# sholtodouglas/RoboticsPlayroomPybullet

Hardware: AMD Instinct MI355X
Metric: env-steps/sec at N=4096 parallel UR5PlayAbsRPY1Obj-v0 envs per MI355X (higher is better)
Workload: dtype f32

## Files before the change

### roboticsplayroompybullet_amd/csrc/rp_kernels.cuh

```cuda
#pragma once
#include <hip/hip_runtime.h>
#include <stdint.h>

#include "rp_device_model.h"
#include "rp_math.cuh"

#define NB_MAX (1 + RP_MAX_ARM + RP_MAX_FREE + RP_MAX_J1)
#define NVP 28
#define MAXC 21
#define MAXACT 64
#define MAXT 4
#define MAXROWC (3 * MAXC + MAXT)
static_assert(MAXACT <= 64 && NB_MAX <= 32, "a candidate record packs its pair index in 6 bits and its bodies in 5 bits each");
#define PM_MAX 11
#define PMC_HDR 4
#define PMC_PT 11
#define PMC_MAN (8 + 4 * PMC_PT)
#define PMC_MANIFOLDS (PMC_HDR + PM_MAX * PMC_MAN)
#define PMC_AX PMC_MANIFOLDS
#define PMC_AXN 16
#define PMC_FLOATS (PMC_MANIFOLDS + 8 * PMC_AXN)
#define RP_MAX_GROUPS 16
#define SORT_KEYS 64
#define SORT_REPS 8
// ... 103 lines not shown
  int act[MAXACT], candn[MAXACT], key[MAXACT];
  float pmu[MAXACT];
  alignas(16) float cand[CANDMAX * 8];
  alignas(16) float Minv[144];
  float tau[RP_MAX_ARM];
  float finv[RP_MAX_FREE * 9];
  float dmu[RP_MAX_OBJ], dmass[RP_MAX_FREE + 1];
  float vstar[32];
  union alignas(16) {
    struct {
      float inert[RP_MAX_ARM * 10], compI[RP_MAX_ARM * 10];
      float vsp[RP_MAX_ARM * 6], csp[RP_MAX_ARM * 6], fsp[RP_MAX_ARM * 6], Fv[RP_MAX_ARM * 6];
      double Md[144];
    };
    struct {
      float srow[MAXSMALL * 8];
      float rowS[3 * PREP_CH * 4], rowT[3 * PREP_CH * 4];
      union {
        struct { float J[3 * PREP_CH * ROWW], B[3 * PREP_CH * ROWW]; };
        float aout[192];
      };
    };
  };
  HULL_POOL_FIELDS
#ifdef RP_LDS_PAD
  float pad[RP_LDS_PAD];
#endif
};
static_assert(offsetof(EnvLds, aabb) % 16 == 0 && offsetof(PrepLds, aabb) % 16 == 0 && offsetof(EnvLds, cand) % 16 == 0 && offsetof(EnvLds, man) % 16 == 0 && offsetof(EnvLds, srow) % 16 == 0 && offsetof(EnvLds, rowS) % 16 == 0 &&
              offsetof(EnvLds, rowT) % 16 == 0 && offsetof(EnvLds, J) % 16 == 0 && offsetof(EnvLds, B) % 16 == 0, "16-byte LDS accesses");
static_assert(sizeof(PrepLds) <= 20480 - 512, "k_prep2: eight blocks (sixteen waves: what its 128 VGPRs allow) per CU");
static_assert(offsetof(PrepLds, roff) % 16 == 0 && offsetof(PrepLds, slot) % 16 == 0 && offsetof(PrepLds, Minv) % 16 == 0 && offsetof(PrepLds, aout) % 16 == 0 &&
              offsetof(PrepLds, Md) % 8 == 0 && offsetof(PrepLds, cand) % 16 == 0 && offsetof(PrepLds, man) % 16 == 0, "16-byte copies out of LDS");

struct __align__(16) ObsLds {
  float st[RP_REC_FLOATS];
  float xR[NB_MAX * 9], xp[NB_MAX * 3];
  float O[4];
  float S[RP_MAX_ARM * 6];
  alignas(16) float cand[2 * 12 * RP_MAX_ARM + 2 * RP_MAX_ARM + 4];
  alignas(16) float out[O_FLOATS];
};
#ifdef RP_CLOCKS
__device__ unsigned long long g_clk[32 * 4096];
#define CLK_MARK(i) if (lane == 0) { g_clk[8 * wb + (i)] = __builtin_readcyclecounter(); }
#if RP_CLOCKS == 2
#define PCLK(i) if (lane == 0) { g_clk[32 * (blockIdx.x & 4095) + (i)] = (i) >= 6 && (i) < 8 ? wall_clock64() : __builtin_readcyclecounter(); }
#define PCLK_ZERO(i) if (lane == 0) { g_clk[32 * (blockIdx.x & 4095) + (i)] = 0ull; }
#define PCLK_ADD(i, v) if (lane == 0) { g_clk[32 * (blockIdx.x & 4095) + (i)] += (unsigned long long)(v); }
#define HCLK_ADD(i, v) if (l16 == 0) { atomicAdd(&g_clk[32 * (blockIdx.x & 4095) + (i)], (unsigned long long)(v)); }
#ifdef RP_HPROF
#define PCLK_G(i, v)
#define PCLK_H(i, v) PCLK_ADD(i, v)
#else
#define PCLK_G(i, v) PCLK_ADD(i, v)
#define PCLK_H(i, v)
#endif
#define CLK_MARK2(i)
#else
#define PCLK(i)
#define PCLK_ZERO(i)
#define PCLK_ADD(i, v)
#define HCLK_ADD(i, v)
#define PCLK_G(i, v)
#define PCLK_H(i, v)
#define CLK_MARK2(i) CLK_MARK(i)
// ... 108 lines not shown

__device__ __forceinline__ Xf joint_compose(const DevModel* m, const Xf& P, int j, float q) {
  Xf r;
  M3 Rj = mul(P.R, ldm3(m->arm_jrot[j]));
  r.p = P.p + mulv(P.R, ld3(m->arm_jpos[j]));
  V3 ax = ld3(m->arm_axis[j]);
  if (m->arm_jtype[j] == 0) {
    r.R = mul(Rj, axis_angle(ax, q));
  } else {
    r.R = Rj;
    r.p = r.p + mulv(Rj, ax) * q;
  }
  return r;
}

template <class LDS>
__device__ __forceinline__ void fk_bodies(const DevModel* m, LDS& L, int lane) {
  float* T = L.cand;
  static_assert(2 * 12 * RP_MAX_ARM + 2 * RP_MAX_ARM <= CANDMAX * 8 && 2 * 12 * RP_MAX_ARM + 2 * RP_MAX_ARM <= (int)(sizeof(L.cand) / sizeof(float)), "fk scratch fits the candidate list");
  int* P = (int*)(T + 2 * 12 * RP_MAX_ARM);
  const int n = m->n_arm;
  Xf x; x.R = ident3(); x.p = mk3(0, 0, 0);
  int par = -1;
  if (lane < n) {
    M3 R0 = ldm3(m->arm_jrot[lane]);
    V3 p0 = ld3(m->arm_jpos[lane]), ax = ld3(m->arm_axis[lane]);
    float q = L.st[ST_Q + lane];
    x.R = R0; x.p = p0;
    if (m->arm_jtype[lane] == 0) x.R = mul(R0, axis_angle(ax, q));
    else x.p = p0 + mulv(R0, ax) * q;
    par = m->arm_parent[lane];
    if (par < 0) { M3 Rb = ldm3(m->base_rot); V3 pb = ld3(m->base_pos); x.p = pb + mulv(Rb, x.p); x.R = mul(Rb, x.R); }
  }
  for (int it = 0; __ballot(par >= 0) != 0ull; it++) {
    float* Tb = T + (it & 1) * 12 * RP_MAX_ARM;
    int* Pb = P + (it & 1) * RP_MAX_ARM;
    if (lane < n) { stm3(&Tb[12 * lane], x.R); st3(&Tb[12 * lane + 9], x.p); Pb[lane] = par; }
    WSYNC();
    if (par >= 0) {
      M3 Ra = ldm3(&Tb[12 * par]); V3 pa = ld3(&Tb[12 * par + 9]);
      x.p = pa + mulv(Ra, x.p); x.R = mul(Ra, x.R);
      par = Pb[par];
    }
  }
  if (lane < n) { stm3(&L.xR[9 * (lane + 1)], x.R); st3(&L.xp[3 * (lane + 1)], x.p); }
  if (lane < m->nbody && !(lane >= 1 && lane <= n)) {
    int b = lane;
    Xf y; y.R = ident3(); y.p = mk3(0, 0, 0);
    if (b > n && b <= n + m->n_free) {
      int k = b - 1 - n;
      const float* f = &L.st[ST_FREE + 13 * k];
      Q4 q = {f[3], f[4], f[5], f[6]};
      y.R = quat_to_m3(q); y.p = ld3(f);
    } else if (b > n + m->n_free) {
      int k = b - 1 - n - m->n_free;
      M3 R0 = ldm3(m->j1_rot[k]);
      V3 ax = ld3(m->j1_axis[k]);
      y.p = ld3(m->j1_pos[k]);
      float q = L.st[ST_JQ + k];
      if (m->j1_type[k] == 0) y.R = mul(R0, axis_angle(ax, q));
      else { y.R = R0; y.p = y.p + mulv(R0, ax) * q; }
    }
    stm3(&L.xR[9 * b], y.R); st3(&L.xp[3 * b], y.p);
  }
}

template <class LDS>
__device__ __forceinline__ void joint_subspaces(const DevModel* m, LDS& L, int lane) {
  if (lane == 0) st3(L.O, ld3(&L.xp[3 * m->site_body[RP_SITE_EE]]));
  WSYNC();
  if (lane < m->n_arm) {
    V3 O = ld3(L.O);
    M3 R = ldm3(&L.xR[9 * (1 + lane)]);
    V3 a = mulv(R, ld3(m->arm_axis[lane]));
    V6 S;
    if (m->arm_jtype[lane] == 0) { S.a = a; S.l = cross(ld3(&L.xp[3 * (1 + lane)]) - O, a); }
    else { S.a = mk3(0, 0, 0); S.l = a; }
    st6(&L.S[6 * lane], S);
  }
}

template <class LDS>
__device__ __forceinline__ void stage_dynamics(const DevModel* m, LDS& L, int t, int env) {
  const int no = m->n_obj, nd = no + m->n_free;
  if (t < nd) {
    const float v = m->dyn[(size_t)env * nd + t];
    if (t < no) L.dmu[t] = v; else L.dmass[t - no] = v;
  }
}
template <class LDS>
__device__ __forceinline__ float pair_friction(const DevModel* m, const LDS& L, int a, int b) {
  return fminf(L.dmu[m->col_obj[a]] * L.dmu[m->col_obj[b]], 10.f);
}
__device__ __forceinline__ V3 ld_wrench(const DevModel* m, int env, int body, int half) {
  return ld3(m->wrench + ((size_t)env * (m->nbody - 1) + body) * 6 + 3 * half);
}
__device__ __forceinline__ bool wrench_on(V3 w) { return w.x != 0.f || w.y != 0.f || w.z != 0.f; }
// ... 965 lines not shown
#pragma unroll
    for (int bit = 0; bit < 3; bit++) {
      const unsigned long long mb = __ballot((npl >> bit) & 1);
      off += __popcll(mb & lower_groups) << bit; tot += __popcll(mb) << bit;
    }
    cbase += tot;
    const int npg = __shfl(np, lane & ~7);
    const int nst = min(npg, max(0, CANDMAX - off));
    if (act && s < nst) {
      float* c = &L.cand[(off + s) * 8];
      *(float4*)c = make_float4(mine.p.x, mine.p.y, mine.p.z, mine.n.x);
      *(float4*)(c + 4) = make_float4(mine.n.y, mine.n.z, mine.dist, __int_as_float(a | (b << 8) | (ai << 16) | (body_a << 22) | (body_b << 27)));
    }
    if (act && s == 0) L.candn[ai] = nst | (min(off, CANDMAX) << 8);
    WSYNC();
  }
  return min(cbase, CANDMAX);
}

__device__ __forceinline__ int manifold_replace_index(const float* c4, const float* pt) {
  int deepest = -1; float maxpen = pt[6];
  for (int i = 0; i < 4; i++) if (c4[8 * i + 6] < maxpen - K_TIE_EPS) { deepest = i; maxpen = c4[8 * i + 6]; }
  float res[4] = {0, 0, 0, 0};
  V3 P = ld3(pt), p0 = ld3(c4), p1 = ld3(c4 + 8), p2 = ld3(c4 + 16), p3 = ld3(c4 + 24), cr;
  if (deepest != 0) { cr = cross(P - p1, p3 - p2); res[0] = dot(cr, cr); }
  if (deepest != 1) { cr = cross(P - p0, p3 - p2); res[1] = dot(cr, cr); }
  if (deepest != 2) { cr = cross(P - p0, p3 - p1); res[2] = dot(cr, cr); }
  if (deepest != 3) { cr = cross(P - p0, p2 - p1); res[3] = dot(cr, cr); }
  int best = 0;
  for (int i = 1; i < 4; i++) if (res[i] > res[best] * (1.f + 1e-4f)) best = i;
  return best;
}

template <class LDS>
__device__ __forceinline__ int collide(const DevModel* m, LDS& L, int lane, int env, const int* npm_early = nullptr) {
  int nact = 0;
  const int npair = m->n_pair;
  const unsigned short* pp = (const unsigned short*)m->pair;
  unsigned short pv[RP_MAX_PAIR / 64];
#pragma unroll
  for (int k = 0; k < RP_MAX_PAIR / 64; k++) { int pi = 64 * k + lane; pv[k] = pp[pi < npair ? pi : 0]; }
  unsigned ovbits = 0u;
#pragma unroll
  for (int k = 0; k < RP_MAX_PAIR / 64; k++) {
    int pi = 64 * k + lane;
    if (64 * k < npair && pi < npair) {
      int a = pv[k] & 255, b = pv[k] >> 8;
      const float4 alo = *(const float4*)&L.aabb[8 * a], ahi = *(const float4*)&L.aabb[8 * a + 4];
      const float4 blo = *(const float4*)&L.aabb[8 * b], bhi = *(const float4*)&L.aabb[8 * b + 4];
      const float margin = fminf(alo.w, blo.w);
      bool sep = (alo.x > bhi.x + margin) | (blo.x > ahi.x + margin) | (alo.y > bhi.y + margin) | (blo.y > ahi.y + margin) | (alo.z > bhi.z + margin) | (blo.z > ahi.z + margin);
      ovbits |= sep ? 0u : (1u << k);
    }
  }
#pragma unroll
  for (int k = 0; k < RP_MAX_PAIR / 64; k++) {
    if (64 * k >= npair) break;
    bool ov = (ovbits >> k) & 1u;
    unsigned long long mask = __ballot(ov);
    int before = __popcll(mask & ((1ull << lane) - 1ull));
    if (ov && nact + before < MAXACT) L.act[nact + before] = 64 * k + lane;
    nact += __popcll(mask);
    if (nact >= MAXACT) { nact = MAXACT; break; }
  }
  WSYNC();
  PCLK(8)
#if defined(RP_CLOCKS) && RP_CLOCKS == 2
  if (lane == 0) g_clk[32 * (blockIdx.x & 4095) + 12] = nact;
#endif
  const int ncand_all = uni(narrowphase_coop<LDS>(m, L, lane, nact, m->persist ? m->pmcache + (size_t)env * PMC_FLOATS + PMC_AX : nullptr));
  WSYNC();
  asm volatile("" : "+v"(lane));
  PCLK(9)
  const unsigned long long lower = (1ull << lane) - 1ull;
  int kept = 0, pk = 0;
  float* man = L.man;
  if (m->persist) {
    float* C = L.npscr + 8 * MANPTS;
    static_assert(8 * MANPTS + PMC_MANIFOLDS <= NPSCR_FLOATS, "the staged contact cache lies behind L.man in the narrowphase scratch");
    float* g = m->pmcache + (size_t)env * PMC_FLOATS;
    const int npm_pre = min(max(uni(npm_early ? *npm_early : __float_as_int(g[0])), 0), PM_MAX);
    const int used_in = PMC_HDR + PMC_MAN * npm_pre;
    for (int i = lane * 4; i < used_in; i += 256) *(float4*)&C[i] = *(const float4*)&g[i];
    if (lane == 0) C[0] = __int_as_float(npm_pre);
    WSYNC();
    PCLK(21)
    int npm = uni(__float_as_int(C[0]));
    {
      const int mykey = lane < npm ? __float_as_int(C[PMC_HDR + PMC_MAN * lane]) : -1;
      const int akey = L.key[lane < nact ? lane : 0];
      bool touched = false; int fl = 0;
      for (int k = 0; k < nact; k++) { const int kk = __builtin_amdgcn_readlane(akey, k); if ((kk & 0xFFFF) == mykey) { touched = true; fl = kk >> 16; } }
      if (touched) C[PMC_HDR + PMC_MAN * lane + 3] = __int_as_float(fl);
      const unsigned long long keep = __ballot(touched);
      WSYNC();
      int nk = 0;
      for (int j = 0; j < npm; j++)
        if ((keep >> j) & 1ull) {
          if (nk != j && lane < PMC_MAN) C[PMC_HDR + PMC_MAN * nk + lane] = C[PMC_HDR + PMC_MAN * j + lane];
          nk++;
        }
      npm = nk;
      WSYNC();
    }
    {
      const int objk = lane < nact ? (L.key[lane] & 0xFFFF) : -1;
      const bool first = lane < nact && (lane == 0 || (L.key[lane - 1] & 0xFFFF) != objk);
      const int mkey = __float_as_int(C[PMC_HDR + PMC_MAN * (lane < npm ? lane : 0)]);
      bool present = false;
      for (int j = 0; j < npm; j++) present |= __builtin_amdgcn_readlane(mkey, j) == objk;
      const bool isnew = first && !present;
      const unsigned long long mnew = __ballot(isnew);
      const int slot = npm + __popcll(mnew & lower);
      if (isnew && slot < PM_MAX) {
        const int pi = L.act[lane];
        float* M = &C[PMC_HDR + PMC_MAN * slot];
        M[0] = __int_as_float(objk); M[1] = __int_as_float(0);
        M[2] = fminf(m->col_margin[m->pair[pi][0]], m->col_margin[m->pair[pi][1]]);
        M[3] = __int_as_float(L.key[lane] >> 16);
        for (int t = 4; t < PMC_MAN; t++) M[t] = 0.f;
      }
      npm = min(PM_MAX, npm + (int)__popcll(mnew));
      WSYNC();
    }
    PCLK(22)
    unsigned long long unmatched, mine = 0ull;
    {
      const int ncand = ncand_all;
      const bool isc = lane < ncand;
      const float* c = &L.cand[8 * (isc ? lane : 0)];
      const V3 p = ld3(c), nr = mk3(c[3], c[4], c[5]);
      const float dist = c[6];
      const int abw = __float_as_int(c[7]);
      const int objk = L.key[(abw >> 16) & 63] & 0xFFFF;
      const int mkey = __float_as_int(C[PMC_HDR + PMC_MAN * (lane < npm ? lane : 0)]);
      int mi = -1;
      for (int jm = 0; jm < npm; jm++) if (__builtin_amdgcn_readlane(mkey, jm) == objk) mi = jm;
      if (!isc) mi = -1;
      const float* M = &C[PMC_HDR + PMC_MAN * (mi >= 0 ? mi : 0)];
      const float thr = M[2];
      if (dist > thr) mi = -1;
      const int n = __float_as_int(M[1]);
      const int ba = (abw >> 22) & 31, bb = (abw >> 27) & 31;
      const V3 lA = tmulv(ldm3(&L.xR[9 * ba]), p + nr * (0.5f * dist) - ld3(&L.xp[3 * ba]));
      const V3 lB = tmulv(ldm3(&L.xR[9 * bb]), p - nr * (0.5f * dist) - ld3(&L.xp[3 * bb]));
      int sl = -1; float shortest = thr * thr;
      for (int q = 0; q < 4; q++) {
        const V3 d = ld3(&M[8 + PMC_PT * q]) - lA;
        const float dd = dot(d, d);
        if (q < n && dd < shortest) { shortest = dd; sl = q; }
      }
      if (lane < 4 * PM_MAX) C[PMC_HDR + PMC_MAN * (lane >> 2) + 4 + (lane & 3)] = 0.f;
      WSYNC();
      const bool hit = mi >= 0 && sl >= 0;
      int* own = (int*)&C[PMC_HDR + PMC_MAN * (hit ? mi : 0) + 4 + (hit ? sl : 0)];
      if (hit) atomicMax(own, lane + 1);
      WSYNC();
      if (hit && *own == lane + 1) {
        float* P = &C[PMC_HDR + PMC_MAN * mi + 8 + PMC_PT * sl];
        st3(P, lA); st3(P + 3, lB); st3(P + 6, nr); P[9] = dist; P[10] = __int_as_float(abw & (int)0xFFC0FFFF);
      }
      unmatched = __ballot(mi >= 0 && sl < 0);
      if (unmatched != 0ull)
        for (int jm = 0; jm < npm; jm++) { const unsigned long long b = __ballot(mi == jm && sl < 0); if (lane == jm) mine = b; }
      WSYNC();
    }
    if (unmatched != 0ull) {
      float* M = &C[PMC_HDR + PMC_MAN * (lane < npm ? lane : 0)];
      int n = __float_as_int(M[1]);
      const float thr = M[2];
      for (unsigned long long todo = lane < npm ? mine : 0ull; __any(todo != 0ull); todo &= todo - 1ull) {
        if (todo == 0ull) continue;
        const int ci = __ffsll((long long)todo) - 1;
        const float* c = &L.cand[8 * ci];
        const int abw = __float_as_int(c[7]);
        const V3 p = ld3(c), nr = mk3(c[3], c[4], c[5]);
        const float dist = c[6];
        const int ba = (abw >> 22) & 31, bb = (abw >> 27) & 31;
// ... 48 lines not shown
      const unsigned d4 = (unsigned)(__ballot(valid && drop) >> (4 * (mi & 15))) & 15u;
      int a0 = 0, a1 = 1, a2 = 2, a3 = 3, nn = n;
      for (int i = n - 1; i >= 0; i--) {
        const int at = i == 0 ? a0 : (i == 1 ? a1 : (i == 2 ? a2 : a3));
        if ((d4 >> at) & 1u) {
          const int last = nn - 1 == 0 ? a0 : (nn - 1 == 1 ? a1 : (nn - 1 == 2 ? a2 : a3));
          if (i == 0) a0 = last; else if (i == 1) a1 = last; else if (i == 2) a2 = last; else a3 = last;
          nn--;
        }
      }
      int slot = -1;
      if (valid && !((d4 >> q) & 1u)) slot = (nn > 0 && a0 == q) ? 0 : ((nn > 1 && a1 == q) ? 1 : ((nn > 2 && a2 == q) ? 2 : ((nn > 3 && a3 == q) ? 3 : -1)));
      const bool single = (fl & 1) != 0;
      bool emit = slot >= 0;
      if (single && nn > 0) {
        const int base = lane & ~3;
        const int s0 = __shfl(slot, base), s1 = __shfl(slot, base + 1), s2 = __shfl(slot, base + 2), s3 = __shfl(slot, base + 3);
        const float e0 = __shfl(dist, base), e1 = __shfl(dist, base + 1), e2 = __shfl(dist, base + 2), e3 = __shfl(dist, base + 3);
        float ds[4] = {0.f, 0.f, 0.f, 0.f}; int who[4] = {0, 0, 0, 0};
        if (s0 >= 0) { ds[s0] = e0; who[s0] = 0; }
        if (s1 >= 0) { ds[s1] = e1; who[s1] = 1; }
        if (s2 >= 0) { ds[s2] = e2; who[s2] = 2; }
        if (s3 >= 0) { ds[s3] = e3; who[s3] = 3; }
        int only = 0;
        for (int k = 1; k < nn; k++) if (ds[k] < ds[only] - K_TIE_EPS) only = k;
        emit = slot >= 0 && who[only] == q;
      }
      cnt = (q == 0 && mine) ? (single ? (nn > 0 ? 1 : 0) : nn) : 0;
      int off = 0;
#pragma unroll
      for (int bit = 0; bit < 3; bit++) off += __popcll(__ballot((cnt >> bit) & 1) & lower) << bit;
      off = __shfl(off, lane & ~3);
      const int room = max(0, MAXC - off);
      if (q == 0 && mine) { kept = min(cnt, room); man = &L.man[8 * (off < MANPTS ? off : 0)]; pk = fl << 16; }
      WSYNC();
      if (slot >= 0) {
        float* P = &C[PMC_HDR + PMC_MAN * mi + 8 + PMC_PT * slot];
#pragma unroll
        for (int t = 0; t < 9; t++) P[t] = pt[t];
        P[9] = dist; P[10] = pt[10];
      }
      if (q == 0 && mine) C[PMC_HDR + PMC_MAN * mi + 1] = __int_as_float(nn);
      const int ri = single ? 0 : slot;
      if (emit && ri < room) {
        const V3 pm = (pA + pB) * 0.5f;
        float* r = &L.man[8 * (off + ri)];
        r[0] = pm.x; r[1] = pm.y; r[2] = pm.z; r[3] = nr.x; r[4] = nr.y; r[5] = nr.z; r[6] = dist; r[7] = __int_as_float(ab);
      }
    }
    WSYNC();
    PCLK(24)
    if (lane == 0) C[0] = __int_as_float(npm);
    WSYNC();
    for (int i = lane * 4; i < PMC_HDR + PMC_MAN * npm; i += 256) *(float4*)&g[i] = *(const float4*)&C[i];
    PCLK(25)
  } else {
  int mycnt = 0, run_end = lane;
  bool single = false;
  if (lane < nact) {
    const int mykey = L.key[lane];
    const bool head = lane == 0 || L.key[lane - 1] != mykey;
    if (head) {
      int sum = 0;
      for (run_end = lane; run_end < nact && L.key[run_end] == mykey; run_end++) sum += L.candn[run_end] & 255;
      single = (mykey & 65536) != 0;
      mycnt = min(sum, single ? 1 : 4);
    }
  }
  int off = 0;
#pragma unroll
  for (int bit = 0; bit < 3; bit++) off += __popcll(__ballot((mycnt >> bit) & 1) & lower) << bit;
  kept = min(mycnt, max(0, MAXC - off));
  man = &L.man[8 * (off < MANPTS ? off : 0)];
  pk = lane < nact ? L.key[lane] : 0;
  if (kept > 0) {
    int cnt = 0;
    for (int j = lane; j < run_end; j++) {
      const int cn = L.candn[j];
      for (int i = 0; i < (cn & 255); i++) {
        const float* c = &L.cand[((cn >> 8) + i) * 8];
        int dst;
        if (single) {
          if (cnt == 0) dst = cnt++;
          else dst = c[6] < man[6] - K_TIE_EPS ? 0 : -1;
        } else if (cnt < 4) dst = cnt++;
        else dst = manifold_replace_index(man, c);
        if (dst >= 0) { const float4 c0 = *(const float4*)c, c1 = *(const float4*)(c + 4); *(float4*)&man[8 * dst] = c0; *(float4*)&man[8 * dst + 4] = c1; }
      }
    }
  }
  WSYNC();
  }
  int cls = 0, key = 0;
  if (kept > 0) { cls = (pk >> 20) & 3; key = 2 * (cls == 2 ? 1 : 0) + ((pk >> 22) & 1); }
  int before = 0, total = 0;
  {
    unsigned long long mk[4];
#pragma unroll
    for (int k = 0; k < 4; k++) mk[k] = __ballot(kept > 0 && key == k);
#pragma unroll
    for (int bit = 0; bit < 3; bit++) {
      const unsigned long long mb = __ballot((kept >> bit) & 1);
      total += __popcll(mb) << bit;
#pragma unroll
      for (int k = 0; k < 4; k++) {
        const int all = __popcll(mb & mk[k]) << bit, low = __popcll(mb & mk[k] & lower) << bit;
        before += k < key ? all : (k == key ? low : 0);
      }
    }
  }
  for (int i = 0; i < kept; i++) {
    const float4 c0 = *(const float4*)&man[8 * i], c1 = *(const float4*)&man[8 * i + 4];
    const int ab = __float_as_int(c1.w);
    const int o = before + i;
    L.conp[3 * o] = c0.x; L.conp[3 * o + 1] = c0.y; L.conp[3 * o + 2] = c0.z;
    L.conn[3 * o] = c0.w; L.conn[3 * o + 1] = c1.x; L.conn[3 * o + 2] = c1.y;
    L.cond[o] = c1.z;
    L.cona[o] = ab & 255; L.conb[o] = (ab >> 8) & 255; L.conk[o] = cls;
    L.conmu[o] = m->persist ? pair_friction(m, L, ab & 255, (ab >> 8) & 255) : L.pmu[(ab >> 16) & 63];
  }
  WSYNC();
  PCLK(10)
  return total;
}

template <class LDS>
__device__ __forceinline__ void arm_dynamics(const DevModel* m, LDS& L, int lane, int env) {
  int n = m->n_arm;
  V3 O = ld3(L.O);
  V3 wf = mk3(0, 0, 0), wt = mk3(0, 0, 0);
  if (lane < n) { wf = ld_wrench(m, env, lane, 0); wt = ld_wrench(m, env, lane, 1); }
  const V3 grav = ld_gravity(m, env);
  if (lane < n) {
    M3 R = ldm3(&L.xR[9 * (1 + lane)]);
    V3 c = ld3(&L.xp[3 * (1 + lane)]) + mulv(R, ld3(m->arm_com[lane])) - O;
    float mass = m->arm_mass[lane];
    M3 Ic = ldm3(m->arm_inertia[lane]);
    M3 Rt; for (int i = 0; i < 3; i++) for (int j = 0; j < 3; j++) Rt.m[3 * i + j] = R.m[3 * j + i];
    M3 Iw = mul(mul(R, Ic), Rt);
    float cc = dot(c, c);
    float* I = &L.inert[10 * lane];
    I[0] = mass; st3(I + 1, c * mass);
    I[4] = Iw.m[0] + mass * (cc - c.x * c.x); I[5] = Iw.m[4] + mass * (cc - c.y * c.y); I[6] = Iw.m[8] + mass * (cc - c.z * c.z);
    I[7] = Iw.m[1] - mass * c.x * c.y; I[8] = Iw.m[2] - mass * c.x * c.z; I[9] = Iw.m[5] - mass * c.y * c.z;
  }
  WSYNC();
  if (lane < n) {
    uint32_t sub = m->arm_sub[lane], anc = m->arm_anc[lane];
    float acc[10];
    for (int k = 0; k < 10; k++) acc[k] = 0.f;
    V6 v = zero6();
    for (int j = 0; j < n; j++) {
// ... 1474 lines not shown
}

__global__ void __launch_bounds__(64) k_action(const DevModel* __restrict__ m, float* __restrict__ state, const float* __restrict__ action,
                                              float* __restrict__ target_poses, int env0, int N, const int* __restrict__ member) {
  action_body(m, state, action, target_poses, env0, N, member, blockIdx.x);
}

__device__ __forceinline__ void copy_out(float* __restrict__ dst, const float* src, int nfloat, int lane) {
  for (int i = lane * 4; i < nfloat; i += 256) *(float4*)(dst + i) = *(const float4*)(src + i);
}

#define NBJ 3
#define LBL_N NBJ
#define NLBL (LBL_N + MAXC)
#define GEAR_LANE 12
#define W3_HDR 0
#define W3_VSTAR 8
#define W3_MU 40
#define W3_MINV 72
#define W3_A 216
#define W3_GEAR (W3_A + 160)
#define W3_ZERO (W3_GEAR + 7)
#define W3_BJ (W3_GEAR + 8)
#define W3_ROWS (W3_BJ + 20)
#define W3_ROWT (W3_ROWS + 4 * MAXROWC)
#define W3_ROFF (W3_ROWT + 4 * MAXROWC)
#define W3_SLOT (W3_ROFF + 64)
#define W3_J (W3_SLOT + 64)
#define W3_B (W3_J + ROWREG)
#define W3_SROW (W3_B + ROWREG)
#define W3_FLOATS (W3_SROW + 4 + 8 * MAXSMALL)
#define STAGE_FLOATS (128 + 2 * ROWREG)
#define AOUT_FLOATS (160 + 8 + 20)
static_assert(W3_A % 4 == 0 && W3_ROWS % 4 == 0 && W3_ROFF % 4 == 0 && AOUT_FLOATS % 4 == 0, "16-byte copies");

#define HV_MAXC 14
#ifndef S4_SLOTS0
#define S4_SLOTS0 8
#endif
#ifndef S4_SLOTS1
#define S4_SLOTS1 8
#endif
__device__ __forceinline__ int hv_class(int nc, int nA, int nB, int nC) {
  const bool heavy = nC != 0 || nA > S4_SLOTS0 || nB > S4_SLOTS1;
  return !heavy ? 0 : (nc <= HV_MAXC ? 1 : 2);
}
#define PREP_THREADS 128
__device__ __forceinline__ void prep2_core(PrepLds& L, const DevModel* __restrict__ m, const float* __restrict__ state, float* __restrict__ ws, const int env, const int cenv,
                                           int* __restrict__ pair_tab, const int pair_idx, int* __restrict__ hv_cnt = nullptr, int* __restrict__ hv_list = nullptr, const int prep_flags = 0) {
  const int tid = threadIdx.x, wid = tid >> 6, lane = tid & 63;
  PCLK(6) PCLK(0) PCLK_ZERO(15) PCLK_ZERO(19) PCLK_ZERO(26) PCLK_ZERO(27) PCLK_ZERO(28) PCLK_ZERO(29) PCLK_ZERO(30) PCLK_ZERO(31)
  static_assert(RP_REC_FLOATS == PREP_THREADS, "one float of the record per thread");
  L.st[tid] = state[(size_t)env * RP_REC_FLOATS + tid];
  if (tid == 64) L.hdr[3] = pair_idx;
  if (tid == 64 && m->persist) L.hdr[2] = __float_as_int(m->pmcache[(size_t)cenv * PMC_FLOATS]);
  stage_dynamics(m, L, tid, cenv);
  __syncthreads();
  PCLK(16)
  if (wid == 0) fk_bodies(m, L, lane);
  __syncthreads();
  PCLK(17)
  float* w = ws + (size_t)env * W3_FLOATS;
  if (wid == 0) {
    collider_aabbs(m, L, lane);
    WSYNC();
    PCLK(1)
    int ncon = collide<PrepLds>(m, L, lane, cenv, &L.hdr[2]);
// ... 17 lines not shown
    WSYNC();
    bool gear = false;
    if (lane < nsmall) {
      const float* s = &L.srow[8 * lane];
      int type = __float_as_int(s[0]), dA = __float_as_int(s[1]);
      float sg = s[2], rhs = s[3], dinv = s[4], lo = s[5], hi = s[6];
      if (type == SR_UNIT) {
        L.aout[dA] = dinv; L.aout[16 + dA] = rhs; L.aout[32 + dA] = lo; L.aout[48 + dA] = hi;
      } else if (type == SR_LIMIT) {
        int pl = sg > 0.f ? 64 : 112;
        L.aout[pl + dA] = sg * rhs; L.aout[pl + 16 + dA] = sg * lo; L.aout[pl + 32 + dA] = sg * hi;
        atomicOr(&L.amask[sg > 0.f ? 0 : 1], 1u << dA);
      } else if (type == SR_J1) {
        int k = lane;
        if (k < NBJ) { float* bq = &L.aout[168]; bq[k] = dinv; bq[4 + k] = rhs; bq[8 + k] = lo; bq[12 + k] = hi; bq[16 + k] = sg; }
      } else {
        float* g = &L.aout[160];
        g[0] = s[1]; g[1] = s[7]; g[2] = sg; g[3] = dinv; g[4] = rhs; g[5] = lo; g[6] = hi;
        gear = true;
      }
    }
    const bool anygear = __ballot(gear) != 0ull;
    if (lane == 0) L.hdr[1] = anygear ? 1 : 0;
    WSYNC();
    if (lane < 32) w[W3_VSTAR + lane] = L.vstar[lane];
    copy_out(w + W3_MINV, L.Minv, 144, lane);
    copy_out(w + W3_A, L.aout, AOUT_FLOATS, lane);
  }
  __syncthreads();
  const int ncon = L.hdr[0];
  int tid_j = threadIdx.x;
  asm volatile("" : "+v"(tid_j));
  const int wid_j = tid_j >> 6;
  if (wid_j == 0) {
    const int lane = tid_j & 63;
    float* w = ws + (size_t)env * W3_FLOATS;
    const int cls = lane < ncon ? L.conk[lane] : 3;
    const unsigned long long mB = __ballot(cls == 0), mA = __ballot(cls == 1), mC = __ballot(cls == 2);
    const unsigned long long lower = (1ull << lane) - 1ull;
    L.slot[lane] = -1;
    L.roff[lane] = 0;
    const int nt = tors_list(m, L, lane, ncon);
    WSYNC();
    if (cls == 0) L.slot[__popcll(mB & lower)] = lane;
    else if (cls == 1) L.slot[21 + __popcll(mA & lower)] = lane;
    else if (cls == 2) L.slot[42 + __popcll(mC & lower)] = lane;
    bool tors_done = nt == 0;
    for (int c0 = 0; c0 < ncon || !tors_done; c0 += PREP_CH) {
      const int nc = max(0, min(PREP_CH, ncon - c0));
      const int ntl = (!tors_done && c0 + PREP_CH >= ncon && 3 * nc + nt <= 3 * PREP_CH) ? nt : 0;
      contact_rows(m, L, lane, c0, nc, ntl);
      WSYNC();
      auto global_row = [&](int lr) { return lr < nc ? c0 + lr : (lr < nc + ntl ? 3 * ncon + (lr - nc) : ncon + 2 * c0 + (lr - nc - ntl)); };
      for (int e = lane; e < (3 * nc + ntl) * ROWW; e += 64) {
        const int lr = e / ROWW, k = e - lr * ROWW;
        const int gr = global_row(lr);
        w[W3_J + gr * ROWW + k] = L.J[e]; w[W3_B + gr * ROWW + k] = L.B[e];
      }
      for (int e = lane; e < (3 * nc + ntl) * 4; e += 64) {
        const int lr = e >> 2, k = e & 3;
        const int gr = global_row(lr);
        float v = L.rowS[e];
        if (k == 3 && lr >= nc && lr < nc + ntl) {
          const int c = L.torc[lr - nc], kc = L.conk[c];
          const unsigned long long mk = kc == 1 ? mA : (kc == 2 ? mC : mB);
          v = __int_as_float(c | (kc << 8) | (__popcll(mk & ((1ull << c) - 1ull)) << 12));
        }
        w[W3_ROWS + gr * 4 + k] = v; w[W3_ROWT + gr * 4 + k] = L.rowT[e];
      }
      if (lane < 3 * nc + ntl && !(lane >= nc && lane < nc + ntl)) {
        const int gr = global_row(lane);
        L.roff[gr] = __float_as_int(L.rowT[4 * lane + 2]) | (__float_as_int(L.rowT[4 * lane + 3]) << 8);
      }
      if (ntl > 0) tors_done = true;
      WSYNC();
    }
    PCLK(4)
    if (lane == 0) {
      int nj = m->n_j1 < NBJ ? m->n_j1 : NBJ;
      w[W3_HDR] = __int_as_float((int)L.amask[0]); w[W3_HDR + 1] = __int_as_float((int)L.amask[1]);
      w[W3_HDR + 2] = __int_as_float(nj); w[W3_HDR + 3] = __int_as_float(ncon);
      w[W3_HDR + 4] = __int_as_float(__popcll(mA)); w[W3_HDR + 5] = __int_as_float(__popcll(mB));
      w[W3_HDR + 6] = __int_as_float(L.hdr[1] | (nt << 8)); w[W3_HDR + 7] = __int_as_float(__popcll(mC));
      if (hv_list != nullptr && (hv_class(ncon, __popcll(mA), __popcll(mB), __popcll(mC)) != 0 || (prep_flags & 1))) hv_list[atomicAdd(hv_cnt, 1)] = env | (ncon << 24);
    }
    if (lane < 32) w[W3_MU + lane] = lane < ncon ? L.conmu[lane] : 0.f;
    copy_out(w + W3_ROFF, (const float*)L.roff, 64, lane);
    copy_out(w + W3_SLOT, (const float*)L.slot, 64, lane);
  } else {
    if ((tid_j & 63) == 0) pair_tab[L.hdr[3]] = env | (ncon << 24);
    if (prep_flags & 1) {
      const int lane = tid_j & 63;
      float* w = ws + (size_t)env * W3_FLOATS;
      const int nsm = (int)L.amask[2];
      if (lane == 0) w[W3_SROW] = __int_as_float(nsm);
      for (int i = lane; i < 8 * nsm; i += 64) w[W3_SROW + 4 + i] = L.srow[i];
    }
  }
  PCLK(5) PCLK(7)
}
__device__ __forceinline__ void prep2_body(const DevModel* __restrict__ m, const float* __restrict__ state, float* __restrict__ ws, int env0, int N,
                                           const int* __restrict__ sort_cnt, int* __restrict__ sort_cnt_next, const int* __restrict__ sort_slot, int* __restrict__ pair_env,
                                           const int* __restrict__ member, const int bid, const int* __restrict__ cache_env = nullptr, int* __restrict__ hv_cnt = nullptr, int* __restrict__ hv_cnt_next = nullptr,
                                           int* __restrict__ hv_list = nullptr, const int prep_flags = 0) {
  __shared__ PrepLds L;
  const int tid = threadIdx.x, wid = tid >> 6, lane = tid & 63;
  int env = env0 + bid;
  if (env >= N) return;
  if (member) env = member[env];
  if (bid == 0) {
    for (int i = tid; i < SORT_BINS; i += PREP_THREADS) sort_cnt_next[i] = 0;
    if (tid == 0 && hv_cnt_next) *hv_cnt_next = 0;
  }
  int pair_place = 0;
  if (wid == 1) {
    const int my_slot = sort_slot[env];
    int cnt8[8];
#pragma unroll
    for (int t = 0; t < 8; t++) cnt8[t] = sort_cnt[8 * lane + t];
    const int mybin = my_slot >> SORT_RANK_BITS;
    int above = 0;
#pragma unroll
    for (int t = 0; t < 8; t++) above += (8 * lane + t > mybin) ? cnt8[t] : 0;
#pragma unroll
    for (int d = 32; d >= 1; d >>= 1) above += __shfl_xor(above, d);
    pair_place = above + (my_slot & SORT_RANK_MASK);
  }
  prep2_core(L, m, state, ws, env, cache_env ? cache_env[env] : env, pair_env, env0 + pair_place, hv_cnt, hv_list ? hv_list + env0 : nullptr, prep_flags);
}
// ... 1517 lines not shown
```

Before: 2.118 million.

## Split prep2 row output across both waves, add steady-state manifold fast path

The prep2 write-out loop now involves both waves of the block. Wave 0 builds the rows, then both waves copy J/B in 8-byte pairs and rowS/rowT as float4 rows, coordinated with block barriers. The persistent-manifold collide path gains a steady-state check that skips compacting and inserting manifolds when nothing changed. It also writes contacts straight into the solver arrays using a factored-out solver_place ranking. Separately, the fk parent-chain loop is moved after the non-arm body setup, and body transforms are loaded earlier. The aim is to cut serial LDS-to-global copy time and per-contact shuffling, at the cost of extra __syncthreads and more complex control flow.

New measurement: 2.142 million, median of 6. 1.1% higher.

```diff
diff --git a/roboticsplayroompybullet_amd/csrc/rp_kernels.cuh b/roboticsplayroompybullet_amd/csrc/rp_kernels.cuh
--- a/roboticsplayroompybullet_amd/csrc/rp_kernels.cuh
+++ b/roboticsplayroompybullet_amd/csrc/rp_kernels.cuh
@@ -159,6 +159,8 @@
 static_assert(sizeof(PrepLds) <= 20480 - 512, "k_prep2: eight blocks (sixteen waves: what its 128 VGPRs allow) per CU");
 static_assert(offsetof(PrepLds, roff) % 16 == 0 && offsetof(PrepLds, slot) % 16 == 0 && offsetof(PrepLds, Minv) % 16 == 0 && offsetof(PrepLds, aout) % 16 == 0 &&
               offsetof(PrepLds, Md) % 8 == 0 && offsetof(PrepLds, cand) % 16 == 0 && offsetof(PrepLds, man) % 16 == 0, "16-byte copies out of LDS");
+static_assert(offsetof(PrepLds, rowS) % 16 == 0 && offsetof(PrepLds, rowT) % 16 == 0 && offsetof(PrepLds, J) % 8 == 0 && offsetof(PrepLds, B) % 8 == 0 && ROWW % 2 == 0,
+              "prep2_core copies rowS / rowT a row (16 bytes) and J / B a pair (8 bytes) at a time");
 
 struct __align__(16) ObsLds {
   float st[RP_REC_FLOATS];
@@ -333,18 +335,6 @@
     par = m->arm_parent[lane];
     if (par < 0) { M3 Rb = ldm3(m->base_rot); V3 pb = ld3(m->base_pos); x.p = pb + mulv(Rb, x.p); x.R = mul(Rb, x.R); }
   }
-  for (int it = 0; __ballot(par >= 0) != 0ull; it++) {
-    float* Tb = T + (it & 1) * 12 * RP_MAX_ARM;
-    int* Pb = P + (it & 1) * RP_MAX_ARM;
-    if (lane < n) { stm3(&Tb[12 * lane], x.R); st3(&Tb[12 * lane + 9], x.p); Pb[lane] = par; }
-    WSYNC();
-    if (par >= 0) {
-      M3 Ra = ldm3(&Tb[12 * par]); V3 pa = ld3(&Tb[12 * par + 9]);
-      x.p = pa + mulv(Ra, x.p); x.R = mul(Ra, x.R);
-      par = Pb[par];
-    }
-  }
-  if (lane < n) { stm3(&L.xR[9 * (lane + 1)], x.R); st3(&L.xp[3 * (lane + 1)], x.p); }
   if (lane < m->nbody && !(lane >= 1 && lane <= n)) {
     int b = lane;
     Xf y; y.R = ident3(); y.p = mk3(0, 0, 0);
@@ -364,6 +354,18 @@
     }
     stm3(&L.xR[9 * b], y.R); st3(&L.xp[3 * b], y.p);
   }
+  for (int it = 0; __ballot(par >= 0) != 0ull; it++) {
+    float* Tb = T + (it & 1) * 12 * RP_MAX_ARM;
+    int* Pb = P + (it & 1) * RP_MAX_ARM;
+    if (lane < n) { stm3(&Tb[12 * lane], x.R); st3(&Tb[12 * lane + 9], x.p); Pb[lane] = par; }
+    WSYNC();
+    if (par >= 0) {
+      M3 Ra = ldm3(&Tb[12 * par]); V3 pa = ld3(&Tb[12 * par + 9]);
+      x.p = pa + mulv(Ra, x.p); x.R = mul(Ra, x.R);
+      par = Pb[par];
+    }
+  }
+  if (lane < n) { stm3(&L.xR[9 * (lane + 1)], x.R); st3(&L.xp[3 * (lane + 1)], x.p); }
 }
 
 template <class LDS>
@@ -1395,6 +1397,26 @@
   return best;
 }
 
+__device__ __forceinline__ int solver_place(const int kept, const int pk, const unsigned long long lower, int& cls, int& before) {
+  int key = 0, total = 0;
+  cls = 0; before = 0;
+  if (kept > 0) { cls = (pk >> 20) & 3; key = 2 * (cls == 2 ? 1 : 0) + ((pk >> 22) & 1); }
+  unsigned long long mk[4];
+#pragma unroll
+  for (int k = 0; k < 4; k++) mk[k] = __ballot(kept > 0 && key == k);
+#pragma unroll
+  for (int bit = 0; bit < 3; bit++) {
+    const unsigned long long mb = __ballot((kept >> bit) & 1);
+    total += __popcll(mb) << bit;
+#pragma unroll
+    for (int k = 0; k < 4; k++) {
+      const int all = __popcll(mb & mk[k]) << bit, low = __popcll(mb & mk[k] & lower) << bit;
+      before += k < key ? all : (k == key ? low : 0);
+    }
+  }
+  return total;
+}
+
 template <class LDS>
 __device__ __forceinline__ int collide(const DevModel* m, LDS& L, int lane, int env, const int* npm_early = nullptr) {
   int nact = 0;
@@ -1436,7 +1458,7 @@
   asm volatile("" : "+v"(lane));
   PCLK(9)
   const unsigned long long lower = (1ull << lane) - 1ull;
-  int kept = 0, pk = 0;
+  int kept = 0, pk = 0, total = 0;
   float* man = L.man;
   if (m->persist) {
     float* C = L.npscr + 8 * MANPTS;
@@ -1449,42 +1471,57 @@
     WSYNC();
     PCLK(21)
     int npm = uni(__float_as_int(C[0]));
+    const int mykey = lane < npm ? __float_as_int(C[PMC_HDR + PMC_MAN * lane]) : -1;
+    const int akey = L.key[lane < nact ? lane : 0];
+    const int pkey = L.key[lane >= 1 && lane < nact ? lane - 1 : 0];
+    bool steady;
+    unsigned long long keep;
     {
-      const int mykey = lane < npm ? __float_as_int(C[PMC_HDR + PMC_MAN * lane]) : -1;
-      const int akey = L.key[lane < nact ? lane : 0];
       bool touched = false; int fl = 0;
       for (int k = 0; k < nact; k++) { const int kk = __builtin_amdgcn_readlane(akey, k); if ((kk & 0xFFFF) == mykey) { touched = true; fl = kk >> 16; } }
       if (touched) C[PMC_HDR + PMC_MAN * lane + 3] = __int_as_float(fl);
-      const unsigned long long keep = __ballot(touched);
-      WSYNC();
-      int nk = 0;
-      for (int j = 0; j < npm; j++)
-        if ((keep >> j) & 1ull) {
-          if (nk != j && lane < PMC_MAN) C[PMC_HDR + PMC_MAN * nk + lane] = C[PMC_HDR + PMC_MAN * j + lane];
-          nk++;
+      keep = __ballot(touched);
+      steady = keep == (1ull << npm) - 1ull;
+      if (steady) {
+        const int objk = lane < nact ? (akey & 0xFFFF) : -1;
+        const bool first = lane < nact && (lane == 0 || (pkey & 0xFFFF) != objk);
+        bool present = false;
+        for (int j = 0; j < npm; j++) present |= __builtin_amdgcn_readlane(mykey, j) == objk;
+        steady = __ballot(first && !present) == 0ull;
+      }
+    }
+    if (!steady) {
+      {
+        WSYNC();
+        int nk = 0;
+        for (int j = 0; j < npm; j++)
+          if ((keep >> j) & 1ull) {
+            if (nk != j && lane < PMC_MAN) C[PMC_HDR + PMC_MAN * nk + lane] = C[PMC_HDR + PMC_MAN * j + lane];
+            nk++;
+          }
+        npm = nk;
+        WSYNC();
+      }
+      {
+        const int objk = lane < nact ? (L.key[lane] & 0xFFFF) : -1;
+        const bool first = lane < nact && (lane == 0 || (L.key[lane - 1] & 0xFFFF) != objk);
+        const int mkey = __float_as_int(C[PMC_HDR + PMC_MAN * (lane < npm ? lane : 0)]);
+        bool present = false;
+        for (int j = 0; j < npm; j++) present |= __builtin_amdgcn_readlane(mkey, j) == objk;
+        const bool isnew = first && !present;
+        const unsigned long long mnew = __ballot(isnew);
+        const int slot = npm + __popcll(mnew & lower);
+        if (isnew && slot < PM_MAX) {
+          const int pi = L.act[lane];
+          float* M = &C[PMC_HDR + PMC_MAN * slot];
+          M[0] = __int_as_float(objk); M[1] = __int_as_float(0);
+          M[2] = fminf(m->col_margin[m->pair[pi][0]], m->col_margin[m->pair[pi][1]]);
+          M[3] = __int_as_float(L.key[lane] >> 16);
+          for (int t = 4; t < PMC_MAN; t++) M[t] = 0.f;
         }
-      npm = nk;
-      WSYNC();
-    }
-    {
-      const int objk = lane < nact ? (L.key[lane] & 0xFFFF) : -1;
-      const bool first = lane < nact && (lane == 0 || (L.key[lane - 1] & 0xFFFF) != objk);
-      const int mkey = __float_as_int(C[PMC_HDR + PMC_MAN * (lane < npm ? lane : 0)]);
-      bool present = false;
-      for (int j = 0; j < npm; j++) present |= __builtin_amdgcn_readlane(mkey, j) == objk;
-      const bool isnew = first && !present;
-      const unsigned long long mnew = __ballot(isnew);
-      const int slot = npm + __popcll(mnew & lower);
-      if (isnew && slot < PM_MAX) {
-        const int pi = L.act[lane];
-        float* M = &C[PMC_HDR + PMC_MAN * slot];
-        M[0] = __int_as_float(objk); M[1] = __int_as_float(0);
-        M[2] = fminf(m->col_margin[m->pair[pi][0]], m->col_margin[m->pair[pi][1]]);
-        M[3] = __int_as_float(L.key[lane] >> 16);
-        for (int t = 4; t < PMC_MAN; t++) M[t] = 0.f;
-      }
-      npm = min(PM_MAX, npm + (int)__popcll(mnew));
-      WSYNC();
+        npm = min(PM_MAX, npm + (int)__popcll(mnew));
+        WSYNC();
+      }
     }
     PCLK(22)
     unsigned long long unmatched, mine = 0ull;
@@ -1496,7 +1533,10 @@
       const float dist = c[6];
       const int abw = __float_as_int(c[7]);
       const int objk = L.key[(abw >> 16) & 63] & 0xFFFF;
-      const int mkey = __float_as_int(C[PMC_HDR + PMC_MAN * (lane < npm ? lane : 0)]);
+      const int ba = (abw >> 22) & 31, bb = (abw >> 27) & 31;
+      const M3 RA = ldm3(&L.xR[9 * ba]), RB = ldm3(&L.xR[9 * bb]);
+      const V3 xA = ld3(&L.xp[3 * ba]), xB = ld3(&L.xp[3 * bb]);
+      const int mkey = steady ? mykey : __float_as_int(C[PMC_HDR + PMC_MAN * (lane < npm ? lane : 0)]);
       int mi = -1;
       for (int jm = 0; jm < npm; jm++) if (__builtin_amdgcn_readlane(mkey, jm) == objk) mi = jm;
       if (!isc) mi = -1;
@@ -1504,9 +1544,8 @@
       const float thr = M[2];
       if (dist > thr) mi = -1;
       const int n = __float_as_int(M[1]);
-      const int ba = (abw >> 22) & 31, bb = (abw >> 27) & 31;
-      const V3 lA = tmulv(ldm3(&L.xR[9 * ba]), p + nr * (0.5f * dist) - ld3(&L.xp[3 * ba]));
-      const V3 lB = tmulv(ldm3(&L.xR[9 * bb]), p - nr * (0.5f * dist) - ld3(&L.xp[3 * bb]));
+      const V3 lA = tmulv(RA, p + nr * (0.5f * dist) - xA);
+      const V3 lB = tmulv(RB, p - nr * (0.5f * dist) - xB);
       int sl = -1; float shortest = thr * thr;
       for (int q = 0; q < 4; q++) {
         const V3 d = ld3(&M[8 + PMC_PT * q]) - lA;
@@ -1621,7 +1660,10 @@
       for (int bit = 0; bit < 3; bit++) off += __popcll(__ballot((cnt >> bit) & 1) & lower) << bit;
       off = __shfl(off, lane & ~3);
       const int room = max(0, MAXC - off);
-      if (q == 0 && mine) { kept = min(cnt, room); man = &L.man[8 * (off < MANPTS ? off : 0)]; pk = fl << 16; }
+      if (q == 0 && mine) { kept = min(cnt, room); pk = fl << 16; }
+      int cls, before;
+      total = solver_place(kept, pk, lower, cls, before);
+      cls = __shfl(cls, lane & ~3); before = __shfl(before, lane & ~3);
       WSYNC();
       if (slot >= 0) {
         float* P = &C[PMC_HDR + PMC_MAN * mi + 8 + PMC_PT * slot];
@@ -1633,8 +1675,11 @@
       const int ri = single ? 0 : slot;
       if (emit && ri < room) {
         const V3 pm = (pA + pB) * 0.5f;
-        float* r = &L.man[8 * (off + ri)];
-        r[0] = pm.x; r[1] = pm.y; r[2] = pm.z; r[3] = nr.x; r[4] = nr.y; r[5] = nr.z; r[6] = dist; r[7] = __int_as_float(ab);
+        const int o = before + ri, ca = ab & 255, cb = (ab >> 8) & 255;
+        st3(&L.conp[3 * o], pm); st3(&L.conn[3 * o], nr);
+        L.cond[o] = dist;
+        L.cona[o] = ca; L.conb[o] = cb; L.conk[o] = cls;
+        L.conmu[o] = pair_friction(m, L, ca, cb);
       }
     }
     WSYNC();
@@ -1679,25 +1724,8 @@
     }
   }
   WSYNC();
-  }
-  int cls = 0, key = 0;
-  if (kept > 0) { cls = (pk >> 20) & 3; key = 2 * (cls == 2 ? 1 : 0) + ((pk >> 22) & 1); }
-  int before = 0, total = 0;
-  {
-    unsigned long long mk[4];
-#pragma unroll
-    for (int k = 0; k < 4; k++) mk[k] = __ballot(kept > 0 && key == k);
-#pragma unroll
-    for (int bit = 0; bit < 3; bit++) {
-      const unsigned long long mb = __ballot((kept >> bit) & 1);
-      total += __popcll(mb) << bit;
-#pragma unroll
-      for (int k = 0; k < 4; k++) {
-        const int all = __popcll(mb & mk[k]) << bit, low = __popcll(mb & mk[k] & lower) << bit;
-        before += k < key ? all : (k == key ? low : 0);
-      }
-    }
-  }
+  int cls, before;
+  total = solver_place(kept, pk, lower, cls, before);
   for (int i = 0; i < kept; i++) {
     const float4 c0 = *(const float4*)&man[8 * i], c1 = *(const float4*)&man[8 * i + 4];
     const int ab = __float_as_int(c1.w);
@@ -1706,7 +1734,8 @@
     L.conn[3 * o] = c0.w; L.conn[3 * o + 1] = c1.x; L.conn[3 * o + 2] = c1.y;
     L.cond[o] = c1.z;
     L.cona[o] = ab & 255; L.conb[o] = (ab >> 8) & 255; L.conk[o] = cls;
-    L.conmu[o] = m->persist ? pair_friction(m, L, ab & 255, (ab >> 8) & 255) : L.pmu[(ab >> 16) & 63];
+    L.conmu[o] = L.pmu[(ab >> 16) & 63];
+  }
   }
   WSYNC();
   PCLK(10)
@@ -3247,7 +3276,8 @@
 #define W3_FLOATS (W3_SROW + 4 + 8 * MAXSMALL)
 #define STAGE_FLOATS (128 + 2 * ROWREG)
 #define AOUT_FLOATS (160 + 8 + 20)
-static_assert(W3_A % 4 == 0 && W3_ROWS % 4 == 0 && W3_ROFF % 4 == 0 && AOUT_FLOATS % 4 == 0, "16-byte copies");
+static_assert(W3_A % 4 == 0 && W3_ROWS % 4 == 0 && W3_ROWT % 4 == 0 && W3_ROFF % 4 == 0 && AOUT_FLOATS % 4 == 0 && W3_FLOATS % 4 == 0, "16-byte copies");
+static_assert(W3_J % 2 == 0 && W3_B % 2 == 0, "8-byte copies of the compact rows");
 
 #define HV_MAXC 14
 #ifndef S4_SLOTS0
@@ -3331,69 +3361,82 @@
   int tid_j = threadIdx.x;
   asm volatile("" : "+v"(tid_j));
   const int wid_j = tid_j >> 6;
-  if (wid_j == 0) {
+  {
     const int lane = tid_j & 63;
     float* w = ws + (size_t)env * W3_FLOATS;
     const int cls = lane < ncon ? L.conk[lane] : 3;
     const unsigned long long mB = __ballot(cls == 0), mA = __ballot(cls == 1), mC = __ballot(cls == 2);
     const unsigned long long lower = (1ull << lane) - 1ull;
-    L.slot[lane] = -1;
-    L.roff[lane] = 0;
-    const int nt = tors_list(m, L, lane, ncon);
-    WSYNC();
-    if (cls == 0) L.slot[__popcll(mB & lower)] = lane;
-    else if (cls == 1) L.slot[21 + __popcll(mA & lower)] = lane;
-    else if (cls == 2) L.slot[42 + __popcll(mC & lower)] = lane;
+    int nt = 0;
+    if (wid_j == 0) {
+      L.slot[lane] = -1;
+      L.roff[lane] = 0;
+      nt = tors_list(m, L, lane, ncon);
+      if (lane == 0) L.amask[3] = (unsigned)nt;
+      WSYNC();
+      if (cls == 0) L.slot[__popcll(mB & lower)] = lane;
+      else if (cls == 1) L.slot[21 + __popcll(mA & lower)] = lane;
+      else if (cls == 2) L.slot[42 + __popcll(mC & lower)] = lane;
+    }
     bool tors_done = nt == 0;
     for (int c0 = 0; c0 < ncon || !tors_done; c0 += PREP_CH) {
+      if (c0 > 0) __syncthreads();
       const int nc = max(0, min(PREP_CH, ncon - c0));
+      if (wid_j == 0) contact_rows(m, L, lane, c0, nc, (!tors_done && c0 + PREP_CH >= ncon && 3 * nc + nt <= 3 * PREP_CH) ? nt : 0);
+      __syncthreads();
+      if (wid_j != 0 && c0 == 0) { nt = (int)L.amask[3]; tors_done = nt == 0; }
       const int ntl = (!tors_done && c0 + PREP_CH >= ncon && 3 * nc + nt <= 3 * PREP_CH) ? nt : 0;
-      contact_rows(m, L, lane, c0, nc, ntl);
+      auto global_row = [&](int lr) { return lr < nc ? c0 + lr : (lr < nc + ntl ? 3 * ncon + (lr - nc) : ncon + 2 * c0 + (lr - nc - ntl)); };
+      const int nrow = 3 * nc + ntl;
+      {
+        static_assert(ROWW % 2 == 0 && PREP_THREADS / (ROWW / 2) == 14 && PREP_THREADS % (ROWW / 2) == 2, "the copy's (row, pair) step");
+        int lr = tid_j / (ROWW / 2), k = tid_j - lr * (ROWW / 2);
+        for (; lr < nrow; ) {
+          const int gr = global_row(lr);
+          *(float2*)&w[W3_J + gr * ROWW + 2 * k] = *(const float2*)&L.J[lr * ROWW + 2 * k];
+          *(float2*)&w[W3_B + gr * ROWW + 2 * k] = *(const float2*)&L.B[lr * ROWW + 2 * k];
+          lr += 14; k += 2;
+          if (k >= ROWW / 2) { k -= ROWW / 2; lr++; }
+        }
+      }
+      if (lane < nrow) {
+        const int gr = global_row(lane);
+        if (wid_j == 0) {
+          float4 v = *(const float4*)&L.rowS[4 * lane];
+          if (lane >= nc && lane < nc + ntl) {
+            const int c = L.torc[lane - nc], kc = L.conk[c];
+            const unsigned long long mk = kc == 1 ? mA : (kc == 2 ? mC : mB);
+            v.w = __int_as_float(c | (kc << 8) | (__popcll(mk & ((1ull << c) - 1ull)) << 12));
+          }
+          *(float4*)&w[W3_ROWS + gr * 4] = v;
+          if (!(lane >= nc && lane < nc + ntl)) L.roff[gr] = __float_as_int(L.rowT[4 * lane + 2]) | (__float_as_int(L.rowT[4 * lane + 3]) << 8);
+        } else {
+          *(float4*)&w[W3_ROWT + gr * 4] = *(const float4*)&L.rowT[4 * lane];
+        }
+      }
+      if (ntl > 0) tors_done = true;
+    }
+    if (wid_j == 0) {
       WSYNC();
-      auto global_row = [&](int lr) { return lr < nc ? c0 + lr : (lr < nc + ntl ? 3 * ncon + (lr - nc) : ncon + 2 * c0 + (lr - nc - ntl)); };
-      for (int e = lane; e < (3 * nc + ntl) * ROWW; e += 64) {
-        const int lr = e / ROWW, k = e - lr * ROWW;
-        const int gr = global_row(lr);
-        w[W3_J + gr * ROWW + k] = L.J[e]; w[W3_B + gr * ROWW + k] = L.B[e];
-      }
-      for (int e = lane; e < (3 * nc + ntl) * 4; e += 64) {
-        const int lr = e >> 2, k = e & 3;
-        const int gr = global_row(lr);
-        float v = L.rowS[e];
-        if (k == 3 && lr >= nc && lr < nc + ntl) {
-          const int c = L.torc[lr - nc], kc = L.conk[c];
-          const unsigned long long mk = kc == 1 ? mA : (kc == 2 ? mC : mB);
-          v = __int_as_float(c | (kc << 8) | (__popcll(mk & ((1ull << c) - 1ull)) << 12));
-        }
-        w[W3_ROWS + gr * 4 + k] = v; w[W3_ROWT + gr * 4 + k] = L.rowT[e];
-      }
-      if (lane < 3 * nc + ntl && !(lane >= nc && lane < nc + ntl)) {
-        const int gr = global_row(lane);
-        L.roff[gr] = __float_as_int(L.rowT[4 * lane + 2]) | (__float_as_int(L.rowT[4 * lane + 3]) << 8);
-      }
-      if (ntl > 0) tors_done = true;
-      WSYNC();
-    }
-    PCLK(4)
-    if (lane == 0) {
-      int nj = m->n_j1 < NBJ ? m->n_j1 : NBJ;
-      w[W3_HDR] = __int_as_float((int)L.amask[0]); w[W3_HDR + 1] = __int_as_float((int)L.amask[1]);
-      w[W3_HDR + 2] = __int_as_float(nj); w[W3_HDR + 3] = __int_as_float(ncon);
-      w[W3_HDR + 4] = __int_as_float(__popcll(mA)); w[W3_HDR + 5] = __int_as_float(__popcll(mB));
-      w[W3_HDR + 6] = __int_as_float(L.hdr[1] | (nt << 8)); w[W3_HDR + 7] = __int_as_float(__popcll(mC));
-      if (hv_list != nullptr && (hv_class(ncon, __popcll(mA), __popcll(mB), __popcll(mC)) != 0 || (prep_flags & 1))) hv_list[atomicAdd(hv_cnt, 1)] = env | (ncon << 24);
-    }
-    if (lane < 32) w[W3_MU + lane] = lane < ncon ? L.conmu[lane] : 0.f;
-    copy_out(w + W3_ROFF, (const float*)L.roff, 64, lane);
-    copy_out(w + W3_SLOT, (const float*)L.slot, 64, lane);
-  } else {
-    if ((tid_j & 63) == 0) pair_tab[L.hdr[3]] = env | (ncon << 24);
-    if (prep_flags & 1) {
-      const int lane = tid_j & 63;
-      float* w = ws + (size_t)env * W3_FLOATS;
-      const int nsm = (int)L.amask[2];
-      if (lane == 0) w[W3_SROW] = __int_as_float(nsm);
-      for (int i = lane; i < 8 * nsm; i += 64) w[W3_SROW + 4 + i] = L.srow[i];
+      PCLK(4)
+      if (lane == 0) {
+        int nj = m->n_j1 < NBJ ? m->n_j1 : NBJ;
+        w[W3_HDR] = __int_as_float((int)L.amask[0]); w[W3_HDR + 1] = __int_as_float((int)L.amask[1]);
+        w[W3_HDR + 2] = __int_as_float(nj); w[W3_HDR + 3] = __int_as_float(ncon);
+        w[W3_HDR + 4] = __int_as_float(__popcll(mA)); w[W3_HDR + 5] = __int_as_float(__popcll(mB));
+        w[W3_HDR + 6] = __int_as_float(L.hdr[1] | (nt << 8)); w[W3_HDR + 7] = __int_as_float(__popcll(mC));
+        if (hv_list != nullptr && (hv_class(ncon, __popcll(mA), __popcll(mB), __popcll(mC)) != 0 || (prep_flags & 1))) hv_list[atomicAdd(hv_cnt, 1)] = env | (ncon << 24);
+      }
+      copy_out(w + W3_ROFF, (const float*)L.roff, 64, lane);
+      copy_out(w + W3_SLOT, (const float*)L.slot, 64, lane);
+    } else {
+      if (lane == 0) pair_tab[L.hdr[3]] = env | (ncon << 24);
+      if (lane < 32) w[W3_MU + lane] = lane < ncon ? L.conmu[lane] : 0.f;
+      if (prep_flags & 1) {
+        const int nsm = (int)L.amask[2];
+        if (lane == 0) w[W3_SROW] = __int_as_float(nsm);
+        for (int i = lane; i < 8 * nsm; i += 64) w[W3_SROW + 4 + i] = L.srow[i];
+      }
     }
   }
   PCLK(5) PCLK(7)
```
